# szaguldo-kamaz/FRI-ReinforcementLearning-C

Hardware: AMD Instinct MI355X
Metric: rule-distance evals/sec (rules x envs) (higher is better)
Workload: dtype f64; 1 GPU; cfg4_acrobot_64k_x_8k_per_gpu; nant=5, universe_len=41, rules_per_env=65536, envs_per_gpu=8192, exact_hits=4, dist_backend=none, world_size=1

## Files before the change

fri-reinforcementlearning-c_amd/__init__.py:

```python
import ctypes as C
import os

PKG_DIR = os.path.dirname(os.path.abspath(__file__))
ROOT = os.path.dirname(PKG_DIR)
HIP_LIB_PATH = os.environ.get("FRIRL_HIP_LIB_OVERRIDE") or os.path.join(PKG_DIR, "lib", "libfrirl_hip.so")

NO_HIT = 0xFFFFFFFF
MAX_NANT = 16
MAX_ACTIONS = 32


class FrirlHipError(RuntimeError):
    pass


class Tables(C.Structure):
    _fields_ = [("nant", C.c_int32), ("U", C.c_int32), ("u", C.c_void_p), ("ve", C.c_void_p)]


class RuleBases(C.Structure):
    _fields_ = [("E", C.c_int32), ("maxR", C.c_int32), ("rb", C.c_void_p), ("nrules", C.c_void_p), ("uidx", C.c_void_p)]


MAX_GRID = 64
# ... 77 lines not shown


class AgentIO(C.Structure):
    _fields_ = [("obs", C.c_void_p), ("q_obs", C.c_void_p), ("reward", C.c_void_p), ("success", C.c_void_p), ("reset", C.c_void_p),
                ("action_out", C.c_void_p), ("action_idx", C.c_void_p)]


class DemonstrationDesc(C.Structure):
    _fields_ = [("T", C.c_int32), ("agent_stride", C.c_int64), ("obs", C.c_void_p), ("q_obs", C.c_void_p), ("action", C.c_void_p),
                ("reward", C.c_void_p), ("success", C.c_void_p), ("start", C.c_void_p), ("length", C.c_void_p)]


class PolicyRowsDesc(C.Structure):
    _fields_ = [("Q", C.c_int32), ("done", C.c_void_p), ("ep_steps", C.c_void_p), ("success", C.c_void_p), ("ep_reward", C.c_void_p),
                ("exclude_mask", C.c_void_p), ("rule_slot", C.c_void_p)]


class PolicyBatchRowsDesc(C.Structure):
    _fields_ = [("n", C.c_int32), ("done", C.c_void_p), ("ep_steps", C.c_void_p), ("success", C.c_void_p), ("ep_reward", C.c_void_p),
                ("row_count", C.c_void_p), ("step_cap", C.c_void_p), ("agents", C.c_void_p), ("nagents", C.c_int32),
                ("exclude_mask", C.c_void_p), ("rule_slot", C.c_void_p), ("rows_live", C.c_void_p)]


class ConvergenceDesc(C.Structure):
    _fields_ = [("prev_nrules", C.c_void_p), ("prev_steps", C.c_void_p), ("prev_reward", C.c_void_p), ("prev_rconc", C.c_void_p),
                ("converged", C.c_void_p), ("episodes", C.c_void_p), ("epended", C.c_void_p)]


_lib = None
_DP = C.POINTER(C.c_double)
LEARN_CHUNK_FN = C.CFUNCTYPE(None, C.c_void_p, C.c_int32, C.c_void_p, C.c_int32)

SIGNATURES = {
    "frirl_hip_version": (C.c_char_p, []),
    "frirl_hip_last_error": (C.c_char_p, []),
    "frirl_hip_device_count": (C.c_int, []),
    "frirl_hip_device_info": (C.c_int, [C.c_int, C.c_char_p, C.c_int, C.POINTER(C.c_int32), C.POINTER(C.c_int64)]),
    "frirl_hip_set_option": (C.c_int, [C.c_char_p, C.c_int]),
    "frirl_hip_get_option": (C.c_int, [C.c_char_p, C.POINTER(C.c_int)]),
    "five_hip_rule_distance_uses_uidx": (C.c_int, [C.c_int32, C.c_int32]),
    "frirl_hip_step_uses_uidx": (C.c_int, [C.c_int32, C.c_int32, C.c_int32, C.c_int32]),
    "five_hip_rule_distance": (C.c_int, [C.POINTER(Tables), C.POINTER(RuleBases), C.c_void_p, C.c_void_p, C.c_void_p, C.c_void_p]),
    "five_hip_rule_distance_packed_words": (C.c_int, [C.c_int32, C.c_int32]),
    "frirl_hip_pack_indices": (C.c_int, [C.POINTER(Tables), C.POINTER(RuleBases), C.c_void_p, C.c_void_p]),
    "five_hip_rule_distance_packed": (C.c_int, [C.POINTER(Tables), C.POINTER(RuleBases), C.c_void_p, C.c_void_p, C.c_void_p, C.c_void_p,
                                                C.c_void_p]),
    "five_hip_rule_distance_packed_workspace_bytes": (C.c_size_t, [C.c_int32, C.c_int32, C.c_int32]),
    "five_hip_rule_distance_packed_ws": (C.c_int, [C.POINTER(Tables), C.POINTER(RuleBases), C.c_void_p, C.c_void_p, C.c_void_p, C.c_void_p,
                                                   C.c_void_p, C.c_size_t, C.c_void_p]),
    "five_hip_rule_distance_coded_bytes": (C.c_size_t, [C.c_int32, C.c_int32, C.c_int32, C.c_int32, C.POINTER(C.c_int32)]),
    "frirl_hip_pack_codes": (C.c_int, [C.POINTER(Tables), C.POINTER(RuleBases), C.c_void_p, C.POINTER(C.c_int32), C.c_void_p, C.c_void_p]),
    "five_hip_rule_distance_coded_ws": (C.c_int, [C.POINTER(Tables), C.POINTER(RuleBases), C.c_void_p, C.c_void_p, C.POINTER(C.c_int32), C.c_void_p,
                                                  C.c_void_p, C.c_void_p, C.c_void_p, C.c_void_p, C.c_size_t, C.c_void_p]),
    "five_hip_sqrt_unscaled_check": (C.c_int, [C.c_void_p, C.c_void_p, C.c_void_p, C.c_int64, C.c_void_p]),
    "five_hip_rule_distance_sq_guard": (C.c_int, [C.POINTER(Tables), C.c_int32, C.c_void_p, C.c_void_p, C.c_void_p]),
    "five_hip_vag_concl": (C.c_int, [C.POINTER(Tables), C.POINTER(RuleBases), C.c_int, C.c_void_p, C.c_void_p, C.c_void_p, C.c_void_p]),
    "five_hip_vag_concl_weight": (C.c_int, [C.POINTER(Tables), C.POINTER(RuleBases), C.c_int, C.c_void_p, C.c_void_p, C.c_void_p, C.c_void_p]),
    "frirl_hip_get_best_action": (C.c_int, [C.POINTER(Tables), C.POINTER(RuleBases), C.c_int, C.c_void_p, C.c_void_p, C.c_int,
                                            C.c_void_p, C.c_void_p, C.c_void_p]),
    "five_hip_shepard_weight_check": (C.c_int, [C.c_void_p, C.c_int64, C.c_int, C.c_int, C.c_void_p, C.c_void_p]),
    "frirl_hip_explore_check": (C.c_int, [C.POINTER(AgentDesc), C.c_int64, C.c_void_p, C.c_void_p, C.c_void_p, C.c_void_p, C.c_void_p, C.c_void_p,
                                          C.c_void_p]),
    "five_hip_vag_concl_shared": (C.c_int, [C.POINTER(Tables), C.POINTER(RuleBases), C.c_int, C.c_int32, C.c_void_p, C.c_void_p, C.c_void_p, C.c_void_p]),
    "frirl_hip_get_best_action_shared": (C.c_int, [C.POINTER(Tables), C.POINTER(RuleBases), C.c_int, C.c_int32, C.c_void_p, C.c_void_p, C.c_int,
                                                   C.c_void_p, C.c_void_p, C.c_void_p]),
    "frirl_hip_rollout_shared": (C.c_int, [C.POINTER(Tables), C.POINTER(RuleBases), C.POINTER(AgentDesc), C.c_int32, C.POINTER(RolloutDesc), C.c_void_p]),
    "frirl_hip_rollout_batch_workspace_bytes": (C.c_size_t, [C.c_int32, C.c_int32, C.c_int32, C.c_int32, C.c_int32]),
    "frirl_hip_rollout_batch": (C.c_int, [C.POINTER(Tables), C.POINTER(RuleBases), C.POINTER(AgentDesc), C.POINTER(RolloutBatchDesc), C.c_void_p,
                                          C.c_void_p, C.c_size_t, C.c_void_p]),
    "frirl_hip_rollout_record": (C.c_int, [C.POINTER(Tables), C.POINTER(RuleBases), C.POINTER(AgentDesc), C.POINTER(RolloutLogDesc), C.c_void_p]),
    "frirl_hip_reduce_shared": (C.c_int, [C.POINTER(Tables), C.POINTER(RuleBases), C.POINTER(AgentDesc), C.c_void_p, C.c_int, C.c_double, C.c_int,
                                          C.POINTER(C.c_int32), C.POINTER(ReduceResult), C.c_void_p]),
    "frirl_hip_reduce_batch_depth": (C.c_int, [C.c_int32, C.c_int32]),
    "frirl_hip_reduce_batch_workspace_bytes": (C.c_size_t, [C.c_int32, C.c_int32, C.c_int32, C.c_int32]),
    "frirl_hip_reduce_batch": (C.c_int, [C.POINTER(Tables), C.POINTER(RuleBases), C.POINTER(AgentDesc), C.c_void_p, C.c_void_p, C.c_void_p, C.c_int,
                                         C.c_double, C.c_int, C.POINTER(C.c_int32), C.POINTER(ReduceResult), C.c_void_p, C.c_size_t, C.c_void_p]),
    "frirl_hip_reduce_walk_check": (C.c_int, [C.c_int, C.POINTER(C.c_int32), _DP, C.c_int, C.c_double, C.c_double, C.c_double,
                                              C.POINTER(C.c_uint32), _DP]),
    "frirl_hip_reduce_batch_starts_depth": (C.c_int, [C.c_int32, C.c_int32, C.c_int32]),
    "frirl_hip_reduce_batch_starts_workspace_bytes": (C.c_size_t, [C.c_int32, C.c_int32, C.c_int32, C.c_int32, C.c_int32]),
    "frirl_hip_reduce_batch_starts": (C.c_int, [C.POINTER(Tables), C.POINTER(RuleBases), C.POINTER(AgentDesc), C.c_void_p, C.POINTER(ReduceStarts),
                                                C.c_void_p, C.c_int, C.c_double, C.c_int, C.POINTER(C.c_int32), C.POINTER(ReduceResult),
                                                C.POINTER(ReduceStartResult), C.c_void_p, C.c_size_t, C.c_void_p]),
    "frirl_hip_reduce_walk_starts_check": (C.c_int, [C.c_int, C.c_int, C.POINTER(C.c_int32), _DP, C.POINTER(C.c_int32), _DP, C.c_double, C.c_double,
                                                     C.POINTER(C.c_uint32)]),
    "frirl_hip_lanes_preferred": (C.c_int, [C.c_int32, C.c_int32, C.c_int32]),
    "frirl_hip_lanes_workspace_bytes": (C.c_size_t, [C.c_int32, C.c_int32, C.c_int32, C.c_int32]),
    "frirl_hip_episode_run_lanes": (C.c_int, [C.POINTER(Tables), C.POINTER(RuleBases), C.POINTER(AgentDesc), C.POINTER(EnvsDesc), C.c_int32,
                                              C.c_void_p, C.c_size_t, C.c_void_p]),
    "frirl_hip_rollout_resident_rules": (C.c_int, [C.c_int32, C.c_int32, C.c_int32, C.c_int32]),
    "frirl_hip_learn_supported": (C.c_int, [C.c_int32, C.c_int32, C.c_int32, C.c_int32, C.c_int32]),
    "frirl_hip_learn_plan": (C.c_int, [C.c_int32, C.c_int32, C.POINTER(C.c_int32), C.POINTER(C.c_int32)]),
    "frirl_hip_learn_workspace_bytes": (C.c_size_t, [C.c_int32, C.c_int32, C.c_int32, C.c_int32]),
    "frirl_hip_learn_run": (C.c_int, [C.POINTER(Tables), C.POINTER(RuleBases), C.POINTER(AgentDesc), C.POINTER(EnvsDesc), C.POINTER(ConvergenceDesc),
                                      C.c_void_p, C.c_int32, C.c_int32, C.c_int32, C.c_void_p, C.c_void_p, C.c_void_p, C.c_size_t, C.c_void_p]),
    "frirl_hip_learn_train_workspace_bytes": (C.c_size_t, [C.c_int32, C.c_int32, C.c_int32, C.c_int32]),
    "frirl_hip_learn_train": (C.c_int, [C.POINTER(Tables), C.POINTER(RuleBases), C.POINTER(AgentDesc), C.POINTER(EnvsDesc), C.POINTER(ConvergenceDesc),
                                        C.c_int32, C.c_int32, C.c_void_p, C.c_void_p, C.c_void_p, C.c_void_p, C.c_size_t, C.POINTER(C.c_int32),
                                        LEARN_CHUNK_FN, C.c_void_p, C.c_void_p]),
    "five_hip_add_rule": (C.c_int, [C.POINTER(Tables), C.POINTER(RuleBases), C.c_void_p, C.c_void_p, C.c_void_p, C.c_void_p, C.c_void_p,
                                    C.c_void_p]),
    "frirl_hip_update_sarsa": (C.c_int, [C.POINTER(Tables), C.POINTER(RuleBases), C.POINTER(AgentDesc), C.POINTER(EnvsDesc), C.c_void_p,
                                         C.c_void_p, C.c_void_p, C.c_void_p, C.c_void_p]),
    "frirl_hip_env_step": (C.c_int, [C.POINTER(AgentDesc), C.c_int32, C.c_int32, C.c_void_p, C.c_void_p, C.c_void_p, C.c_void_p, C.c_void_p,
                                     C.c_void_p, C.c_void_p]),
    "frirl_hip_episode_begin": (C.c_int, [C.POINTER(Tables), C.POINTER(RuleBases), C.POINTER(AgentDesc), C.POINTER(EnvsDesc), C.c_void_p]),
# ... 106 lines not shown
            fn = getattr(L, name)
            fn.restype, fn.argtypes = res, args
        _lib = L
    return _lib


def check(rc, what=""):
    if rc != 0:
        raise FrirlHipError(f"{what}: rc={rc}: {lib().frirl_hip_last_error().decode()}")


def set_option(name, value):
    old = C.c_int()
    check(lib().frirl_hip_get_option(name.encode(), C.byref(old)), "frirl_hip_get_option")
    check(lib().frirl_hip_set_option(name.encode(), int(value)), "frirl_hip_set_option")
    return old.value


def _ptr(t):
    return None if t is None else C.c_void_p(t.data_ptr())


def _stream(stream=None):
    import torch
    s = stream if stream is not None else torch.cuda.current_stream()
    return C.c_void_p(s.cuda_stream)


class Problem:

    def __init__(self, u, ve, rb, nrules, uidx=None):
        import torch
        assert u.is_cuda and ve.is_cuda and rb.is_cuda and nrules.is_cuda
        assert u.dtype == torch.float64 and ve.dtype == torch.float64 and rb.dtype == torch.float64 and nrules.dtype == torch.int32
        self.nant, self.U = u.shape
        self.E, cols, self.maxR = rb.shape
        assert cols == self.nant + 1 and ve.shape == u.shape and nrules.shape == (self.E,)
        self.u, self.ve, self.rb, self.nrules = u.contiguous(), ve.contiguous(), rb.contiguous(), nrules.contiguous()
        self.uidx = None
        if uidx is not None:
            assert uidx.is_cuda and uidx.dtype == torch.int16 and uidx.shape == (self.E, self.nant, self.maxR) and self.U <= 32767
            self.uidx = uidx.contiguous()
        self.tables = Tables(self.nant, self.U, self.u.data_ptr(), self.ve.data_ptr())
        self._bases = RuleBases(self.E, self.maxR, self.rb.data_ptr(), self.nrules.data_ptr(),
                                self.uidx.data_ptr() if self.uidx is not None else None)
        self.pidx = None
        self._pidx_key = None
        W = lib().five_hip_rule_distance_packed_words(self.nant, self.U) if self.uidx is not None else 0
        if W > 0:
            self.pidx = torch.empty((self.E, W, self.maxR), dtype=torch.int32, device=self.uidx.device)
            self._pack(None)
        self.codes = self._code_dict = self._code_rank = self._code_d = None
        self._codes_key = None
        if self.pidx is not None and self.nant <= 5:
            self._pack_codes(None)
        self._rd_ws = {}
        self._ro_ws = {}

    @property
    def bases(self):
        self._pidx_key = None
        self._codes_key = None
        return self._bases

    def _pack(self, stream):
        check(lib().frirl_hip_pack_indices(C.byref(self.tables), C.byref(self._bases), _ptr(self.pidx), _stream(stream)),
              "frirl_hip_pack_indices")
        self._pidx_key = (self.uidx.data_ptr(), self.uidx._version)

    def _pidx_current(self, stream):
        if self._pidx_key != (self.uidx.data_ptr(), self.uidx._version):
            self._pack(stream)
        return self.pidx

    def _pack_codes(self, stream):
        import torch
        dev = self.uidx.device
        with torch.cuda.stream(stream if stream is not None else torch.cuda.current_stream()):
            nr = self.nrules.to(torch.int64)
            upto = (nr + (nr & 1)).clamp(max=self.maxR)
            cols = torch.arange(self.maxR, device=dev)
            dimoff = (65 * torch.arange(self.nant, device=dev)).view(1, self.nant, 1)
            counts = torch.zeros((self.nant * 65,), dtype=torch.int64, device=dev)
            step = max(1, (1 << 26) // (self.nant * self.maxR))
            for e0 in range(0, self.E, step):
                v = self.uidx[e0:e0 + step].to(torch.int64) & 63
                live = (cols.view(1, -1) < upto[e0:e0 + step].view(-1, 1)).unsqueeze(1)
                v = torch.where(live, v, torch.full_like(v, 64)) + dimoff
                counts += torch.bincount(v.flatten(), minlength=self.nant * 65)
            present = counts.view(self.nant, 65)[:, :64] > 0
            rank = (present.cumsum(1) - 1).clamp(min=0).to(torch.uint8).contiguous()
            idx = torch.arange(64, device=dev).expand(self.nant, 64)
            dct = torch.where(present, idx, torch.full_like(idx, 255)).sort(1).values.to(torch.uint8).contiguous()
            d = present.sum(1).clamp(min=1).to(torch.int32).cpu().tolist()
        darr = (C.c_int32 * self.nant)(*d)
        n = lib().five_hip_rule_distance_coded_bytes(self.nant, self.U, self.E, self.maxR, darr)
        if n:
            if self.codes is None or self.codes.numel() != n:
                self.codes = torch.empty((n,), dtype=torch.uint8, device=dev)
            self._code_dict, self._code_rank, self._code_d = dct, rank, darr
            check(lib().frirl_hip_pack_codes(C.byref(self.tables), C.byref(self._bases), _ptr(rank), darr, _ptr(self.codes), _stream(stream)),
                  "frirl_hip_pack_codes")
        else:
            self.codes = self._code_dict = self._code_rank = self._code_d = None
        self._codes_key = (self.uidx.data_ptr(), self.uidx._version, self.nrules.data_ptr(), self.nrules._version)

    def _codes_current(self, stream):
        if self.nant <= 5 and self._codes_key != (self.uidx.data_ptr(), self.uidx._version, self.nrules.data_ptr(), self.nrules._version):
            self._pack_codes(stream)
        return self.codes

    def _rd_workspace(self, stream):
        import torch
        key = _stream(stream).value
        if key not in self._rd_ws:
            n = lib().five_hip_rule_distance_packed_workspace_bytes(self.nant, self.U, self.E)
            self._rd_ws[key] = torch.empty((n,), dtype=torch.uint8, device=self.pidx.device) if n else None
        return self._rd_ws[key]

    def rule_distance(self, x, ruledists=None, hit=None, materialise=True, stream=None):
        import torch
        assert x.is_cuda and x.dtype == torch.float64 and x.shape == (self.E, self.nant) and x.is_contiguous()
        if materialise and ruledists is None:
            ruledists = torch.empty((self.E, self.maxR), dtype=torch.float64, device=x.device)
        if hit is None:
            hit = torch.empty((self.E,), dtype=torch.int32, device=x.device)
        if self.pidx is not None and self._codes_current(stream) is not None:
            ws = self._rd_workspace(stream)
            rc = lib().five_hip_rule_distance_coded_ws(C.byref(self.tables), C.byref(self._bases), _ptr(self.codes), _ptr(self._code_dict), self._code_d,
                                                       _ptr(self._pidx_current(stream)), _ptr(x), _ptr(ruledists) if materialise else None,
                                                       _ptr(hit), _ptr(ws), ws.numel() if ws is not None else 0, _stream(stream))
            check(rc, "five_hip_rule_distance_coded_ws")
        elif self.pidx is not None:
            ws = self._rd_workspace(stream)
            rc = lib().five_hip_rule_distance_packed_ws(C.byref(self.tables), C.byref(self._bases), _ptr(self._pidx_current(stream)), _ptr(x),
                                                        _ptr(ruledists) if materialise else None, _ptr(hit), _ptr(ws),
                                                        ws.numel() if ws is not None else 0, _stream(stream))
            check(rc, "five_hip_rule_distance_packed_ws")
        else:
            rc = lib().five_hip_rule_distance(C.byref(self.tables), C.byref(self._bases), _ptr(x),
                                              _ptr(ruledists) if materialise else None, _ptr(hit), _stream(stream))
            check(rc, "five_hip_rule_distance")
        return (ruledists if materialise else None), hit

    def vag_concl(self, x, p=0, stream=None):
        import torch
        assert x.is_cuda and x.dtype == torch.float64 and x.shape == (self.E, self.nant) and x.is_contiguous()
        conc = torch.empty((self.E,), dtype=torch.float64, device=x.device)
        hit = torch.empty((self.E,), dtype=torch.int32, device=x.device)
        check(lib().five_hip_vag_concl(C.byref(self.tables), C.byref(self._bases), p, _ptr(x), _ptr(conc), _ptr(hit), _stream(stream)),
              "five_hip_vag_concl")
        return conc, hit

    def vag_concl_weight(self, x, p=0, weights=None, stream=None):
        import torch
        assert x.is_cuda and x.dtype == torch.float64 and x.shape == (self.E, self.nant) and x.is_contiguous()
        if weights is None:
            weights = torch.full((self.E, self.maxR), float("nan"), dtype=torch.float64, device=x.device)
        hit = torch.empty((self.E,), dtype=torch.int32, device=x.device)
        check(lib().five_hip_vag_concl_weight(C.byref(self.tables), C.byref(self._bases), p, _ptr(x), _ptr(weights), _ptr(hit),
                                              _stream(stream)), "five_hip_vag_concl_weight")
        return weights, hit

    def get_best_action(self, states, action_ve, p=0, stream=None):
        import torch
        assert states.is_cuda and states.dtype == torch.float64 and states.shape == (self.E, self.nant - 1) and states.is_contiguous()
        A = action_ve.numel()
        actconc = torch.empty((self.E, A), dtype=torch.float64, device=states.device)
        best = torch.empty((self.E,), dtype=torch.int32, device=states.device)
        check(lib().frirl_hip_get_best_action(C.byref(self.tables), C.byref(self._bases), p, _ptr(states), _ptr(action_ve), A,
                                              _ptr(actconc), _ptr(best), _stream(stream)), "frirl_hip_get_best_action")
        return actconc, best

    def vag_concl_shared(self, x, p=0, stream=None):
        import torch
        assert self.E == 1 and x.is_cuda and x.dtype == torch.float64 and x.shape[1] == self.nant and x.is_contiguous()
        Q = x.shape[0]
        conc = torch.empty((Q,), dtype=torch.float64, device=x.device)
        hit = torch.empty((Q,), dtype=torch.int32, device=x.device)
        check(lib().five_hip_vag_concl_shared(C.byref(self.tables), C.byref(self._bases), p, Q, _ptr(x), _ptr(conc), _ptr(hit), _stream(stream)),
              "five_hip_vag_concl_shared")
        return conc, hit

    def get_best_action_shared(self, states, action_ve, p=0, stream=None):
        import torch
        assert self.E == 1 and states.is_cuda and states.dtype == torch.float64 and states.shape[1] == self.nant - 1 and states.is_contiguous()
        Q, A = states.shape[0], action_ve.numel()
        actconc = torch.empty((Q, A), dtype=torch.float64, device=states.device)
        best = torch.empty((Q,), dtype=torch.int32, device=states.device)
        check(lib().frirl_hip_get_best_action_shared(C.byref(self.tables), C.byref(self._bases), p, Q, _ptr(states), _ptr(action_ve), A, _ptr(actconc),
                                                     _ptr(best), _stream(stream)), "frirl_hip_get_best_action_shared")
# ... 899 lines not shown
```

fri-reinforcementlearning-c_amd/csrc/five_rule_distance.hip:

```cpp
#include <stdlib.h>

#include <type_traits>

#include "device_common.h"

namespace frirl {

__device__ __forceinline__ void item_to_env_chunk(unsigned item, int cpe, int E, bool env_fastest, int &e, int &c)
{
    if (env_fastest) { c = (int)(item / (unsigned)E); e = (int)(item - (unsigned)c * (unsigned)E); }
    else { e = (int)(item / (unsigned)cpe); c = (int)(item - (unsigned)e * (unsigned)cpe); }
}

template <int NANT, bool WRITE, int UNROLL, int NT>
__global__ __launch_bounds__(FRIRL_BLOCK) void rule_distance_kernel(
    const double *__restrict__ u, const double *__restrict__ ve, int U, const double *__restrict__ rb,
    const int32_t *__restrict__ nrules, int maxR, const double *__restrict__ x, double *__restrict__ dists,
    uint32_t *__restrict__ hit, int rules_per_block, int cpe, int E, int env_fastest)
{
    int e, c;
    item_to_env_chunk(blockIdx.x, cpe, E, env_fastest != 0, e, c);
    const int R = nrules[e];
    const int r0 = c * rules_per_block;
    if (r0 >= R) return;
// ... 959 lines not shown
#pragma unroll
        for (int j = 0; j < 4; j++) {
            const int rr = r + j * STEP;
            if (rr < r_end) {
                const double a0 = cd_rule_sq<NANT>(code[2 * j], sq_s, cs), a1 = cd_rule_sq<NANT>(code[2 * j + 1], sq_s, cs);
                const bool z0 = FAST ? a0 == 0.0 : __dsqrt_rn(a0) == 0.0, z1 = FAST ? a1 == 0.0 : __dsqrt_rn(a1) == 0.0;
                if (z1 && rr + 1 < R) best = min(best, (unsigned)(rr + 1));
                if (z0) best = min(best, (unsigned)rr);
            }
        }
        return best;
    };
    if (any) {
        code[0] = w[0].x << 3;
        code[1] = __builtin_amdgcn_alignbit(w[0].y, w[0].x, 21);
        code[2] = __builtin_amdgcn_alignbit(w[1].x, w[0].y, 13);
        code[3] = w[1].x >> 5;
        code[4] = w[1].y << 3;
        code[5] = __builtin_amdgcn_alignbit(w[2].x, w[1].y, 21);
        code[6] = __builtin_amdgcn_alignbit(w[2].y, w[2].x, 13);
        code[7] = w[2].y >> 5;
        if (fast) sweep(std::true_type{});
        else sweep(std::false_type{});
    }
    if (!__any(lo == 0u)) return;
    unsigned best = FRIRL_HIP_NO_HIT;
    if (any) best = fast ? first_hit(std::true_type{}) : first_hit(std::false_type{});
    best = wave_min_u32(best);
    if ((threadIdx.x & (FRIRL_WAVE - 1)) == 0 && best != FRIRL_HIP_NO_HIT) atomicMin(&hit[e], best);
}

template <int NANT>
static int launch_coded(const frirl_hip_tables *t, const frirl_hip_rulebases *b, const uint8_t *codes, const uint8_t *dict, const CodeParams &cp,
                        const double *x, double *ruledists, uint32_t *hit, void *ws, hipStream_t s)
{
    using namespace frirl_host;
    const long cpe = ((long)b->maxR + RD_CD_TILE - 1) / RD_CD_TILE;
    if (cpe * ((long)b->E + RD_XCDS) > 0x7FFFFFFFL) { set_error("five_hip_rule_distance_coded_ws: too many work items"); return FRIRL_HIP_EINVAL; }
    double *sqtab = static_cast<double *>(ws);
    uint32_t *fastv = reinterpret_cast<uint32_t *>(sqtab + (size_t)b->E * NANT * (1 << RD_PK_BITS));
    const unsigned items = (unsigned)cpe * (unsigned)((b->E + RD_XCDS - 1) / RD_XCDS * RD_XCDS);
    const GroupDiv gd = group_div((uint32_t)(RD_XCDS * cpe));
    hipLaunchKernelGGL((sq_tables_kernel<NANT, RD_PK_BITS, true>), dim3((unsigned)((b->E + FRIRL_WAVES_PER_BLOCK - 1) / FRIRL_WAVES_PER_BLOCK)), dim3(FRIRL_BLOCK),
                       0, s, t->u, t->ve, t->U, b->E, x, sqtab, fastv, hit, dict);
    if (ruledists)
        hipLaunchKernelGGL((rule_distance_cd_kernel<NANT, true>), dim3(items), dim3(FRIRL_BLOCK), 0, s, codes, b->nrules, b->maxR, ruledists, hit, (int)cpe,
                           b->E, sqtab, fastv, cp, gd);
    else
        hipLaunchKernelGGL((rule_distance_cd_kernel<NANT, false>), dim3(items), dim3(FRIRL_BLOCK), 0, s, codes, b->nrules, b->maxR, ruledists, hit, (int)cpe,
                           b->E, sqtab, fastv, cp, gd);
    return check_launch("five_hip_rule_distance_coded_ws");
}

__global__ void sqrt_unscaled_check_kernel(const double *__restrict__ a, double *__restrict__ fast, double *__restrict__ ref, long n)
{
    const long i = (long)blockIdx.x * blockDim.x + threadIdx.x;
    if (i >= n) return;
    fast[i] = sqrt_unscaled(a[i]);
    ref[i] = __dsqrt_rn(a[i]);
}

template <int NANT>
__global__ __launch_bounds__(FRIRL_BLOCK) void sq_guard_kernel(const double *__restrict__ u, const double *__restrict__ ve, int U,
                                                             const double *__restrict__ x, int32_t *__restrict__ ok)
{
    constexpr int TS = 1 << RD_PK_BITS;
    __shared__ double sq_s[NANT * TS];
    __shared__ double q_s[NANT];
    const int e = blockIdx.x;
    double tv[(NANT * TS + FRIRL_BLOCK - 1) / FRIRL_BLOCK];
    load_sq_sources<NANT, RD_PK_BITS, FRIRL_BLOCK>(ve, U, tv, (int)threadIdx.x);
    if (threadIdx.x < NANT) q_s[threadIdx.x] = observe_ve(u, ve, U, threadIdx.x, x[(size_t)e * NANT + threadIdx.x]);
    __syncthreads();
    const bool fast = !__syncthreads_or(!fill_sq_table<NANT, RD_PK_BITS, FRIRL_BLOCK>(q_s, sq_s, tv, (int)threadIdx.x));
    if (threadIdx.x == 0) ok[e] = fast ? 1 : 0;
}

}

extern "C" int five_hip_rule_distance_uses_uidx(int32_t nant, int32_t U)
{
    return nant >= 1 && nant <= FRIRL_HIP_MAX_NANT && U <= 65536 && sizeof(double) * nant * (size_t)U <= 150 * 1024 && !frirl_host::opts().no_uidx;
}

extern "C" int five_hip_rule_distance(const frirl_hip_tables *t, const frirl_hip_rulebases *b, const double *x,
                                      double *ruledists, uint32_t *hit, void *stream)
{
    using namespace frirl_host;
    int rc = check_rulebases(t, b);
    if (rc) return rc;
    if (!x || !hit) { set_error("five_hip_rule_distance: NULL x/hit"); return FRIRL_HIP_EINVAL; }
    if (ruledists && (reinterpret_cast<uintptr_t>(ruledists) & 15)) { set_error("five_hip_rule_distance: ruledists must be 16-byte aligned"); return FRIRL_HIP_EINVAL; }
    if ((rc = check_device())) return rc;
    hipStream_t s = as_stream(stream);

    switch (t->nant) {
#define FRIRL_CASE(N) case N: return frirl::launch_nant<N>(t, b, x, ruledists, hit, s);
        FRIRL_CASE(1) FRIRL_CASE(2) FRIRL_CASE(3) FRIRL_CASE(4) FRIRL_CASE(5) FRIRL_CASE(6) FRIRL_CASE(7) FRIRL_CASE(8)
        FRIRL_CASE(9) FRIRL_CASE(10) FRIRL_CASE(11) FRIRL_CASE(12) FRIRL_CASE(13) FRIRL_CASE(14) FRIRL_CASE(15) FRIRL_CASE(16)
#undef FRIRL_CASE
    }
    set_error("five_hip_rule_distance: unsupported nant=%d", t->nant);
    return FRIRL_HIP_EINVAL;
}

extern "C" int five_hip_rule_distance_packed_words(int32_t nant, int32_t U)
// ... 110 lines not shown
    using namespace frirl_host;
    int rc = check_rulebases(t, b);
    if (rc) return rc;
    if (!b->uidx || !rank || !codes) { set_error("frirl_hip_pack_codes: NULL uidx/rank/codes"); return FRIRL_HIP_EINVAL; }
    frirl::CodeParams cp;
    if (!frirl::coded_bytes(t->nant, t->U, b->E, b->maxR, d) || !frirl::code_params(t->nant, d, cp)) {
        set_error("frirl_hip_pack_codes: nant=%d U=%d with these dictionary lengths is not served by the coded form", t->nant, t->U);
        return FRIRL_HIP_EINVAL;
    }
    if (reinterpret_cast<uintptr_t>(codes) & 7) { set_error("frirl_hip_pack_codes: codes must be 8-byte aligned"); return FRIRL_HIP_EINVAL; }
    if ((rc = check_device())) return rc;
    const int tpe = (b->maxR + frirl::RD_CD_TILE - 1) / frirl::RD_CD_TILE;
    const long ntiles = (long)b->E * tpe;
    long grid = ntiles;
    if (grid > (long)frirl::device_cus() * 32) grid = (long)frirl::device_cus() * 32;
    hipLaunchKernelGGL(frirl::pack_codes_kernel, dim3((unsigned)grid), dim3(FRIRL_BLOCK), 0, as_stream(stream), b->uidx, b->nrules, t->nant, b->maxR, tpe,
                       ntiles, rank, cp, codes);
    return check_launch("frirl_hip_pack_codes");
}

extern "C" int five_hip_rule_distance_coded_ws(const frirl_hip_tables *t, const frirl_hip_rulebases *b, const uint8_t *codes, const uint8_t *dict,
                                               const int32_t *d, const uint32_t *pidx, const double *x, double *ruledists, uint32_t *hit,
                                               void *workspace, size_t workspace_bytes, void *stream)
{
    using namespace frirl_host;
    int rc = check_rulebases(t, b);
    if (rc) return rc;
    const Options &o = opts();
    const bool plain = !o.rd_coded || !o.rd_packed || !o.rd_sqdiff || !o.rd_prepass || o.rd_persist == 1 || o.no_uidx || o.rd_order != 0 ||
                       (o.rd_unroll != 0 && o.rd_unroll != 4) || (o.rd_chunk != 0 && o.rd_chunk != frirl::RD_CD_TILE);
    frirl::CodeParams cp;
    if (plain || !frirl::coded_bytes(t->nant, t->U, b->E, b->maxR, d) || !frirl::code_params(t->nant, d, cp))
        return five_hip_rule_distance_packed_ws(t, b, pidx, x, ruledists, hit, workspace, workspace_bytes, stream);
    const size_t need = frirl::packed_ws_bytes(t->nant, t->U, b->E);
    if (!workspace || workspace_bytes < need) {
        set_error("five_hip_rule_distance_coded_ws: workspace of %zu B at %p, nant=%d U=%d E=%d needs %zu B "
                  "(five_hip_rule_distance_packed_workspace_bytes)", workspace_bytes, workspace, t->nant, t->U, b->E, need);
        return FRIRL_HIP_EINVAL;
    }
    if (reinterpret_cast<uintptr_t>(workspace) & 15) { set_error("five_hip_rule_distance_coded_ws: workspace must be 16-byte aligned"); return FRIRL_HIP_EINVAL; }
    if (!codes || !dict || !x || !hit) { set_error("five_hip_rule_distance_coded_ws: NULL codes/dict/x/hit"); return FRIRL_HIP_EINVAL; }
    if (reinterpret_cast<uintptr_t>(codes) & 7) { set_error("five_hip_rule_distance_coded_ws: codes must be 8-byte aligned"); return FRIRL_HIP_EINVAL; }
    if (ruledists && (reinterpret_cast<uintptr_t>(ruledists) & 15)) { set_error("five_hip_rule_distance_coded_ws: ruledists must be 16-byte aligned"); return FRIRL_HIP_EINVAL; }
    if ((rc = check_device())) return rc;
    hipStream_t s = as_stream(stream);
    switch (t->nant) {
#define FRIRL_CASE(N) case N: return frirl::launch_coded<N>(t, b, codes, dict, cp, x, ruledists, hit, workspace, s);
        FRIRL_CASE(1) FRIRL_CASE(2) FRIRL_CASE(3) FRIRL_CASE(4) FRIRL_CASE(5)
#undef FRIRL_CASE
    }
    set_error("five_hip_rule_distance_coded_ws: unsupported nant=%d", t->nant);
    return FRIRL_HIP_EINVAL;
}
```

include/frirl_hip.h:

```cpp
#ifndef FRIRL_HIP_H
#define FRIRL_HIP_H

#include <stdint.h>

#ifdef __cplusplus
extern "C" {
#endif

#define FRIRL_HIP_MAX_NANT     16
#define FRIRL_HIP_MAX_ACTIONS  32
#define FRIRL_HIP_MAX_GRID     64
#define FRIRL_HIP_NO_HIT       0xFFFFFFFFu

#define FRIRL_HIP_ENV_MOUNTAINCAR 0
#define FRIRL_HIP_ENV_CARTPOLE    1
#define FRIRL_HIP_ENV_ACROBOT     2
#define FRIRL_HIP_ENV_EXTERNAL    3

#define FRIRL_HIP_UPD_INACTIVE   0
#define FRIRL_HIP_UPD_EXACT      1
#define FRIRL_HIP_UPD_SPREAD     2
#define FRIRL_HIP_UPD_INSERTED   3
#define FRIRL_HIP_UPD_SKIPPED    4
#define FRIRL_HIP_UPD_FULL       5

#define FRIRL_HIP_OK        0
#define FRIRL_HIP_ENODEV   -1
#define FRIRL_HIP_EINVAL   -2
#define FRIRL_HIP_ELAUNCH  -3

typedef struct frirl_hip_tables {
    int32_t nant;
    int32_t U;
    const double *u;
    const double *ve;
} frirl_hip_tables;

typedef struct frirl_hip_rulebases {
    int32_t E;
    int32_t maxR;
    double *rb;
    int32_t *nrules;
    uint16_t *uidx;
} frirl_hip_rulebases;

const char *frirl_hip_version(void);
const char *frirl_hip_last_error(void);
int frirl_hip_device_count(void);
int frirl_hip_device_info(int device, char *name, int name_len, int32_t *cus, int64_t *hbm_bytes);

int frirl_hip_set_option(const char *name, int value);
int frirl_hip_get_option(const char *name, int *value);
int five_hip_rule_distance_uses_uidx(int32_t nant, int32_t U);
int frirl_hip_step_uses_uidx(int32_t nant, int32_t U, int32_t maxR, int32_t E);

int five_hip_rule_distance(const frirl_hip_tables *t, const frirl_hip_rulebases *b, const double *x,
                           double *ruledists, uint32_t *hit, void *stream);

int five_hip_rule_distance_packed_words(int32_t nant, int32_t U);
int frirl_hip_pack_indices(const frirl_hip_tables *t, const frirl_hip_rulebases *b, uint32_t *pidx, void *stream);
int five_hip_rule_distance_packed(const frirl_hip_tables *t, const frirl_hip_rulebases *b, const uint32_t *pidx, const double *x,
                                  double *ruledists, uint32_t *hit, void *stream);
size_t five_hip_rule_distance_packed_workspace_bytes(int32_t nant, int32_t U, int32_t E);
int five_hip_rule_distance_packed_ws(const frirl_hip_tables *t, const frirl_hip_rulebases *b, const uint32_t *pidx, const double *x,
                                     double *ruledists, uint32_t *hit, void *workspace, size_t workspace_bytes, void *stream);
size_t five_hip_rule_distance_coded_bytes(int32_t nant, int32_t U, int32_t E, int32_t maxR, const int32_t *d);
int frirl_hip_pack_codes(const frirl_hip_tables *t, const frirl_hip_rulebases *b, const uint8_t *rank, const int32_t *d, uint8_t *codes,
                         void *stream);
int five_hip_rule_distance_coded_ws(const frirl_hip_tables *t, const frirl_hip_rulebases *b, const uint8_t *codes, const uint8_t *dict,
                                    const int32_t *d, const uint32_t *pidx, const double *x, double *ruledists, uint32_t *hit,
                                    void *workspace, size_t workspace_bytes, void *stream);
int five_hip_sqrt_unscaled_check(const double *a, double *fast, double *ref, int64_t n, void *stream);
int five_hip_rule_distance_sq_guard(const frirl_hip_tables *t, int32_t E, const double *x, int32_t *ok, void *stream);

int five_hip_vag_concl(const frirl_hip_tables *t, const frirl_hip_rulebases *b, int p, const double *x,
                       double *conc, uint32_t *hit, void *stream);

int five_hip_vag_concl_weight(const frirl_hip_tables *t, const frirl_hip_rulebases *b, int p, const double *x,
                              double *weights, uint32_t *hit, void *stream);

int frirl_hip_get_best_action(const frirl_hip_tables *t, const frirl_hip_rulebases *b, int p, const double *states,
                              const double *action_ve, int A, double *actconc, int32_t *best, void *stream);

int five_hip_shepard_weight_check(const double *s, int64_t n, int p, int form, double *w, void *stream);

typedef struct frirl_hip_agent {
    double alpha, gamma;
    double qdiff_pos_boundary;
    double qdiff_neg_boundary;
    double weight_significant;
    int32_t skip_rules;
    int32_t p;
    int32_t A;
    int32_t env_kind;
    int32_t max_steps;
    int32_t no_random;
    int32_t grid_len[FRIRL_HIP_MAX_NANT];
    double grid_div[FRIRL_HIP_MAX_NANT];
    double values_def[FRIRL_HIP_MAX_NANT];
    const double *grid_values;
    const double *action_ve;
    double epsilon;
    double reward_good_above;
    double qdiff_final_tolerance;
    uint64_t seed;
    int32_t evaluate;
    int32_t debug_flags;
    uint64_t env_id_base;
} frirl_hip_agent;

int frirl_hip_explore_check(const frirl_hip_agent *agent, int64_t n, const uint32_t *env, const uint32_t *episode, const uint32_t *step,
                            const int32_t *greedy, int32_t *out_action, double *out_unit, void *stream);

typedef struct frirl_hip_rollout {
    const double *start_states;
    const uint32_t *exclude_mask;
    const uint8_t *rule_slot;
    int32_t *steps;
    double *reward;
    int32_t *success;
    double *final_states;
} frirl_hip_rollout;
int frirl_hip_rollout_shared(const frirl_hip_tables *t, const frirl_hip_rulebases *b, const frirl_hip_agent *agent, int32_t Q,
                             const frirl_hip_rollout *ro, void *stream);
// ... 349 lines not shown
```

Measured before the change: 545.5 billion evals/s.

## Add wide dictionary-coded rule-distance path for larger per-dimension tables

Adds a new coded form for rule bases whose value tables exceed the small-table limit. Each rule's per-dimension dictionary ranks are packed into 48-bit codes, three 64-bit words per thread covering four rules. A persistent kernel with an atomic work counter and a prefetched next item reads these codes and looks up distances from an LDS table. The aim is to shrink the bytes streamed per rule compared with int16 index reads. The cost is an extra packing kernel, a per-call hipMallocAsync, and more dispatch complexity; it only applies when the table size falls in the wide window and the earlier packed path is not taken.

```diff
diff --git a/fri-reinforcementlearning-c_amd/__init__.py b/fri-reinforcementlearning-c_amd/__init__.py
--- a/fri-reinforcementlearning-c_amd/__init__.py
+++ b/fri-reinforcementlearning-c_amd/__init__.py
@@ -153,6 +153,11 @@
     "frirl_hip_pack_codes": (C.c_int, [C.POINTER(Tables), C.POINTER(RuleBases), C.c_void_p, C.POINTER(C.c_int32), C.c_void_p, C.c_void_p]),
     "five_hip_rule_distance_coded_ws": (C.c_int, [C.POINTER(Tables), C.POINTER(RuleBases), C.c_void_p, C.c_void_p, C.POINTER(C.c_int32), C.c_void_p,
                                                   C.c_void_p, C.c_void_p, C.c_void_p, C.c_void_p, C.c_size_t, C.c_void_p]),
+    "five_hip_rule_distance_wide_bytes": (C.c_size_t, [C.c_int32, C.c_int32, C.c_int32, C.c_int32, C.POINTER(C.c_int32)]),
+    "five_hip_rule_distance_wide_fields": (C.c_int, [C.c_int32, C.c_int32, C.POINTER(C.c_int32), C.POINTER(C.c_uint32), C.POINTER(C.c_uint32)]),
+    "frirl_hip_pack_wide": (C.c_int, [C.POINTER(Tables), C.POINTER(RuleBases), C.c_void_p, C.POINTER(C.c_int32), C.c_void_p, C.c_void_p]),
+    "five_hip_rule_distance_wide": (C.c_int, [C.POINTER(Tables), C.POINTER(RuleBases), C.c_void_p, C.c_void_p, C.POINTER(C.c_int32), C.c_void_p,
+                                              C.c_void_p, C.c_void_p, C.c_void_p]),
     "five_hip_sqrt_unscaled_check": (C.c_int, [C.c_void_p, C.c_void_p, C.c_void_p, C.c_int64, C.c_void_p]),
     "five_hip_rule_distance_sq_guard": (C.c_int, [C.POINTER(Tables), C.c_int32, C.c_void_p, C.c_void_p, C.c_void_p]),
     "five_hip_vag_concl": (C.c_int, [C.POINTER(Tables), C.POINTER(RuleBases), C.c_int, C.c_void_p, C.c_void_p, C.c_void_p, C.c_void_p]),
@@ -365,6 +370,8 @@
             self._pack(None)
         self.codes = self._code_dict = self._code_rank = self._code_d = None
         self._codes_key = None
+        ones = (C.c_int32 * self.nant)(*([1] * self.nant))
+        self._wide = self.uidx is not None and lib().five_hip_rule_distance_wide_bytes(self.nant, self.U, self.E, self.maxR, ones) > 0
         if self.pidx is not None and self.nant <= 5:
             self._pack_codes(None)
         self._rd_ws = {}
@@ -389,31 +396,35 @@
     def _pack_codes(self, stream):
         import torch
         dev = self.uidx.device
+        W = self.U if self._wide else 64
+        small, none = (torch.int16, 0x7FFF) if self._wide else (torch.uint8, 255)
         with torch.cuda.stream(stream if stream is not None else torch.cuda.current_stream()):
             nr = self.nrules.to(torch.int64)
             upto = (nr + (nr & 1)).clamp(max=self.maxR)
             cols = torch.arange(self.maxR, device=dev)
-            dimoff = (65 * torch.arange(self.nant, device=dev)).view(1, self.nant, 1)
-            counts = torch.zeros((self.nant * 65,), dtype=torch.int64, device=dev)
+            dimoff = ((W + 1) * torch.arange(self.nant, device=dev)).view(1, self.nant, 1)
+            counts = torch.zeros((self.nant * (W + 1),), dtype=torch.int64, device=dev)
             step = max(1, (1 << 26) // (self.nant * self.maxR))
             for e0 in range(0, self.E, step):
-                v = self.uidx[e0:e0 + step].to(torch.int64) & 63
+                v = self.uidx[e0:e0 + step].to(torch.int64)
+                v = v.clamp(0, W - 1) if self._wide else v & 63
                 live = (cols.view(1, -1) < upto[e0:e0 + step].view(-1, 1)).unsqueeze(1)
-                v = torch.where(live, v, torch.full_like(v, 64)) + dimoff
-                counts += torch.bincount(v.flatten(), minlength=self.nant * 65)
-            present = counts.view(self.nant, 65)[:, :64] > 0
-            rank = (present.cumsum(1) - 1).clamp(min=0).to(torch.uint8).contiguous()
-            idx = torch.arange(64, device=dev).expand(self.nant, 64)
-            dct = torch.where(present, idx, torch.full_like(idx, 255)).sort(1).values.to(torch.uint8).contiguous()
+                v = torch.where(live, v, torch.full_like(v, W)) + dimoff
+                counts += torch.bincount(v.flatten(), minlength=self.nant * (W + 1))
+            present = counts.view(self.nant, W + 1)[:, :W] > 0
+            rank = (present.cumsum(1) - 1).clamp(min=0).to(small).contiguous()
+            idx = torch.arange(W, device=dev).expand(self.nant, W)
+            dct = torch.where(present, idx, torch.full_like(idx, none)).sort(1).values.to(small).contiguous()
             d = present.sum(1).clamp(min=1).to(torch.int32).cpu().tolist()
         darr = (C.c_int32 * self.nant)(*d)
-        n = lib().five_hip_rule_distance_coded_bytes(self.nant, self.U, self.E, self.maxR, darr)
+        size, pack = ((lib().five_hip_rule_distance_wide_bytes, lib().frirl_hip_pack_wide) if self._wide else
+                      (lib().five_hip_rule_distance_coded_bytes, lib().frirl_hip_pack_codes))
+        n = size(self.nant, self.U, self.E, self.maxR, darr)
         if n:
             if self.codes is None or self.codes.numel() != n:
                 self.codes = torch.empty((n,), dtype=torch.uint8, device=dev)
             self._code_dict, self._code_rank, self._code_d = dct, rank, darr
-            check(lib().frirl_hip_pack_codes(C.byref(self.tables), C.byref(self._bases), _ptr(rank), darr, _ptr(self.codes), _stream(stream)),
-                  "frirl_hip_pack_codes")
+            check(pack(C.byref(self.tables), C.byref(self._bases), _ptr(rank), darr, _ptr(self.codes), _stream(stream)), pack.__name__)
         else:
             self.codes = self._code_dict = self._code_rank = self._code_d = None
         self._codes_key = (self.uidx.data_ptr(), self.uidx._version, self.nrules.data_ptr(), self.nrules._version)
@@ -450,6 +461,10 @@
                                                         _ptr(ruledists) if materialise else None, _ptr(hit), _ptr(ws),
                                                         ws.numel() if ws is not None else 0, _stream(stream))
             check(rc, "five_hip_rule_distance_packed_ws")
+        elif self._wide and self._codes_current(stream) is not None:
+            rc = lib().five_hip_rule_distance_wide(C.byref(self.tables), C.byref(self._bases), _ptr(self.codes), _ptr(self._code_dict), self._code_d,
+                                                   _ptr(x), _ptr(ruledists) if materialise else None, _ptr(hit), _stream(stream))
+            check(rc, "five_hip_rule_distance_wide")
         else:
             rc = lib().five_hip_rule_distance(C.byref(self.tables), C.byref(self._bases), _ptr(x),
                                               _ptr(ruledists) if materialise else None, _ptr(hit), _stream(stream))
diff --git a/fri-reinforcementlearning-c_amd/csrc/five_rule_distance.hip b/fri-reinforcementlearning-c_amd/csrc/five_rule_distance.hip
--- a/fri-reinforcementlearning-c_amd/csrc/five_rule_distance.hip
+++ b/fri-reinforcementlearning-c_amd/csrc/five_rule_distance.hip
@@ -1035,6 +1035,224 @@
     return check_launch("five_hip_rule_distance_coded_ws");
 }
 
+static constexpr int RD_WD_BLOCK = 512, RD_WD_TILE = 2 * RD_WD_BLOCK * 2, RD_WD_TILE_BYTES = 6 * RD_WD_TILE, RD_WD_PIECE = 8 * RD_WD_BLOCK;
+static constexpr int RD_WD_MAX_NANT = 5, RD_WD_MAX_BITS = 48;
+
+struct WideParams {
+    uint32_t shift[RD_WD_MAX_NANT], bits[RD_WD_MAX_NANT], d[RD_WD_MAX_NANT];
+};
+
+static bool wide_shape(int nant, int U)
+{
+    if (nant < 1 || nant > RD_WD_MAX_NANT || U < 1) return false;
+    const size_t tab_bytes = sizeof(double) * (size_t)nant * (size_t)U;
+    return tab_bytes > RD_SMALL_TABLE_BYTES && tab_bytes <= 64 * 1024;
+}
+
+static int wide_params(int nant, int U, const int32_t *d, WideParams &wp)
+{
+    if (!wide_shape(nant, U) || !d) return 0;
+    int total = 0, na = 0;
+    for (int k = 0; k < RD_WD_MAX_NANT; k++) wp.shift[k] = wp.bits[k] = 0u, wp.d[k] = 1u;
+    for (int k = 0; k < nant; k++) {
+        if (d[k] < 1 || d[k] > U) return 0;
+        const int bits = ceil_log2((uint32_t)d[k]);
+        wp.shift[k] = (uint32_t)total;
+        wp.bits[k] = (uint32_t)bits;
+        wp.d[k] = (uint32_t)d[k];
+        total += bits;
+        if (total <= 32) na = k + 1;
+    }
+    return total <= RD_WD_MAX_BITS ? na : 0;
+}
+
+static size_t wide_bytes(int nant, int U, long E, long maxR, const int32_t *d)
+{
+    WideParams wp;
+    if (E < 1 || maxR < 2 || !wide_params(nant, U, d, wp)) return 0;
+    return (size_t)E * (size_t)((maxR + RD_WD_TILE - 1) / RD_WD_TILE) * RD_WD_TILE_BYTES;
+}
+
+__global__ __launch_bounds__(RD_WD_BLOCK) void pack_wide_kernel(const uint16_t *__restrict__ uidx, const int32_t *__restrict__ nrules, int nant, int U, int maxR,
+                                                                int tpe, long ntiles, const uint16_t *__restrict__ rank, WideParams wp,
+                                                                uint8_t *__restrict__ codes)
+{
+    const int t = threadIdx.x;
+    for (long tile = blockIdx.x; tile < ntiles; tile += gridDim.x) {
+        const long e = tile / tpe;
+        const int c = (int)(tile - e * tpe);
+        const int R = nrules[e];
+        const int Rp = min(R + (R & 1), maxR);
+        const uint16_t *__restrict__ src = uidx + (size_t)e * nant * maxR;
+        uint64_t code[4];
+#pragma unroll
+        for (int i = 0; i < 4; i++) {
+            const int r = c * RD_WD_TILE + 2 * t + (i & 1) + 2 * RD_WD_BLOCK * (i >> 1);
+            uint64_t v = 0u;
+            if (r < Rp) {
+                for (int k = 0; k < nant; k++) {
+                    const uint32_t i_k = min((uint32_t)src[(size_t)k * maxR + r], (uint32_t)(U - 1));
+                    v |= (uint64_t)rank[k * U + i_k] << wp.shift[k];
+                }
+            }
+            code[i] = v & ((1ull << RD_WD_MAX_BITS) - 1ull);
+        }
+        uint64_t *__restrict__ dst = reinterpret_cast<uint64_t *>(codes + (size_t)tile * RD_WD_TILE_BYTES + 8 * t);
+        dst[0] = code[0] | code[1] << 48;
+        dst[RD_WD_PIECE / 8] = code[1] >> 16 | code[2] << 32;
+        dst[2 * (RD_WD_PIECE / 8)] = code[2] >> 32 | code[3] << 16;
+    }
+}
+
+template <int NANT, int NA>
+struct WideScan {
+    uint32_t off[NANT], bits[NANT];
+    __device__ __forceinline__ explicit WideScan(const WideParams &wp)
+    {
+#pragma unroll
+        for (int k = 0; k < NANT; k++) off[k] = k < NA ? wp.shift[k] : wp.shift[k] - 16u, bits[k] = wp.bits[k];
+    }
+};
+
+template <int NANT, int NA>
+__device__ __forceinline__ double2 wide_pair_distance(uint32_t a0, uint32_t b0, uint32_t a1, uint32_t b1, const double (&q)[NANT],
+                                                      const double *__restrict__ tab_s, int U, const WideScan<NANT, NA> &ws)
+{
+    double a0s = 0.0, a1s = 0.0;
+#pragma unroll
+    for (int k = 0; k < NANT; k++) {
+        const double *__restrict__ row = tab_s + k * U;
+        const double t0 = row[__builtin_amdgcn_ubfe(k < NA ? a0 : b0, ws.off[k], ws.bits[k])];
+        const double t1 = row[__builtin_amdgcn_ubfe(k < NA ? a1 : b1, ws.off[k], ws.bits[k])];
+        const double d0 = q[k] - t0, d1 = q[k] - t1;
+        const double s0 = d0 * d0, s1 = d1 * d1;
+        a0s = k == 0 ? s0 : a0s + s0;
+        a1s = k == 0 ? s1 : a1s + s1;
+    }
+    double2 d;
+    d.x = __dsqrt_rn(a0s);
+    d.y = __dsqrt_rn(a1s);
+    return d;
+}
+
+template <int NANT, int NA, bool WRITE>
+__global__ __launch_bounds__(RD_WD_BLOCK) void rule_distance_wide_persist_kernel(
+    const double *__restrict__ ve, int U, const uint16_t *__restrict__ dict, const uint8_t *__restrict__ codes, const int32_t *__restrict__ nrules,
+    int maxR, const double *__restrict__ qv, double *__restrict__ dists, uint32_t *__restrict__ hit, int cpe, int nitems,
+    unsigned *__restrict__ counter, WideParams wp)
+{
+    extern __shared__ double tab_s[];
+    __shared__ int batch_s[2];
+    constexpr int BLOCK = RD_WD_BLOCK, KB = 4, STEP = BLOCK * 2;
+    const int nbatches = (nitems + KB - 1) / KB;
+    u32x2_t w[3];
+    double qn[NANT];
+    int en = 0, cn = 0, Rn = 0;
+    auto load_item = [&](int it) {
+        en = it / cpe; cn = it - en * cpe;
+        Rn = nrules[en];
+        if (cn * RD_WD_TILE + 2 * (int)threadIdx.x < Rn) {
+            const uint8_t *__restrict__ src = codes + (size_t)it * RD_WD_TILE_BYTES + 8 * threadIdx.x;
+#pragma unroll
+            for (int m = 0; m < 3; m++) w[m] = __builtin_nontemporal_load(reinterpret_cast<const u32x2_t *>(src + m * RD_WD_PIECE));
+        }
+#pragma unroll
+        for (int k = 0; k < NANT; k++) qn[k] = qv[(size_t)en * NANT + k];
+    };
+    int slot = 0, sub = 0;
+    if (threadIdx.x == 0) batch_s[0] = (int)atomicAdd(counter, 1u);
+    __syncthreads();
+    int batch = batch_s[0];
+    int item = batch < nbatches ? batch * KB : nitems;
+    if (item < nitems) load_item(item);
+#pragma unroll
+    for (int k = 0; k < NANT; k++)
+        for (int j = threadIdx.x; j < (int)wp.d[k]; j += BLOCK) tab_s[k * U + j] = ve[k * U + min((int)dict[k * U + j], U - 1)];
+    const WideScan<NANT, NA> ws(wp);
+    __syncthreads();
+    while (item < nitems) {
+        const int e = en, c = cn, R = Rn;
+        u32x2_t cw[3];
+        double q[NANT];
+#pragma unroll
+        for (int m = 0; m < 3; m++) cw[m] = w[m];
+#pragma unroll
+        for (int k = 0; k < NANT; k++) q[k] = qn[k];
+        int nxt;
+        sub++;
+        if (sub < KB && item + 1 < nitems) nxt = item + 1;
+        else {
+            sub = 0;
+            slot ^= 1;
+            if (threadIdx.x == 0) batch_s[slot] = (int)atomicAdd(counter, 1u);
+            __syncthreads();
+            batch = batch_s[slot];
+            nxt = batch < nbatches ? batch * KB : nitems;
+        }
+        if (nxt < nitems) load_item(nxt);
+        double *__restrict__ out = WRITE ? dists + (size_t)e * maxR : nullptr;
+        const int r = c * RD_WD_TILE + 2 * (int)threadIdx.x;
+        unsigned best = FRIRL_HIP_NO_HIT;
+#pragma unroll
+        for (int j = 0; j < 2; j++) {
+            const int rr = r + j * STEP;
+            if (rr < R) {
+                const uint32_t x0 = j == 0 ? cw[0].x : cw[1].y, x1 = j == 0 ? cw[0].y : cw[2].x, x2 = j == 0 ? cw[1].x : cw[2].y;
+                const double2 d = wide_pair_distance<NANT, NA>(x0, __builtin_amdgcn_alignbit(x1, x0, 16), __builtin_amdgcn_alignbit(x2, x1, 16), x2,
+                                                               q, tab_s, U, ws);
+                if (WRITE) { __builtin_nontemporal_store(d.x, out + rr); __builtin_nontemporal_store(d.y, out + rr + 1); }
+                if (d.y == 0.0 && rr + 1 < R) best = min(best, (unsigned)(rr + 1));
+                if (d.x == 0.0) best = min(best, (unsigned)rr);
+            }
+        }
+        if (best != FRIRL_HIP_NO_HIT) atomicMin(&hit[e], best);
+        item = nxt;
+    }
+}
+
+template <int NANT, int NA>
+static int launch_wide(const frirl_hip_tables *t, const frirl_hip_rulebases *b, const uint8_t *codes, const uint16_t *dict, const WideParams &wp,
+                       const double *x, double *ruledists, uint32_t *hit, hipStream_t s)
+{
+    using namespace frirl_host;
+    const size_t tab_bytes = sizeof(double) * NANT * (size_t)t->U;
+    const long cpe = ((long)b->maxR + RD_WD_TILE - 1) / RD_WD_TILE;
+    const long nitems = cpe * (long)b->E;
+    if (nitems > 0x7FFFFFF0L) { set_error("five_hip_rule_distance_wide: %ld work items exceed the 31-bit item index", nitems); return FRIRL_HIP_EINVAL; }
+    const long nbatches = (nitems + 3) / 4;
+    const int wgs = 3 * (tab_bytes + 256) <= 160 * 1024 ? 3 : 2;
+    long grid = (long)device_cus() * wgs;
+    if (grid > nbatches) grid = nbatches;
+    const size_t qv_off = 256, bytes = qv_off + sizeof(double) * (size_t)b->E * NANT;
+    void *scratch = nullptr;
+    hipError_t e1 = hipMallocAsync(&scratch, bytes, s);
+    if (e1 != hipSuccess) { (void)hipGetLastError(); set_error("five_hip_rule_distance_wide: hipMallocAsync(%zu B) failed: %s", bytes, hipGetErrorString(e1)); return FRIRL_HIP_ELAUNCH; }
+    unsigned *counter = static_cast<unsigned *>(scratch);
+    double *qv = reinterpret_cast<double *>(static_cast<char *>(scratch) + qv_off);
+    const int nq = b->E * NANT;
+    hipLaunchKernelGGL(observe_reset_kernel, dim3((nq + 255) / 256), dim3(256), 0, s, t->u, t->ve, t->U, NANT, b->E, x, qv, hit, counter);
+    auto launch = [&](auto k) {
+        e1 = hipFuncSetAttribute(reinterpret_cast<const void *>(k), hipFuncAttributeMaxDynamicSharedMemorySize, (int)tab_bytes);
+        if (e1 == hipSuccess) hipLaunchKernelGGL(k, dim3((unsigned)grid), dim3(RD_WD_BLOCK), tab_bytes, s, t->ve, t->U, dict, codes, b->nrules, b->maxR, qv, ruledists, hit, (int)cpe, (int)nitems, counter, wp);
+    };
+    if (ruledists) launch(rule_distance_wide_persist_kernel<NANT, NA, true>);
+    else launch(rule_distance_wide_persist_kernel<NANT, NA, false>);
+    const hipError_t e2 = hipFreeAsync(scratch, s);
+    if (e1 != hipSuccess) { set_error("five_hip_rule_distance_wide: cannot reserve %zu B of LDS: %s", tab_bytes, hipGetErrorString(e1)); return FRIRL_HIP_ELAUNCH; }
+    if (e2 != hipSuccess) { set_error("five_hip_rule_distance_wide: hipFreeAsync failed: %s", hipGetErrorString(e2)); return FRIRL_HIP_ELAUNCH; }
+    return check_launch("five_hip_rule_distance_wide");
+}
+
+template <int NANT, int NA = NANT>
+static int launch_wide_na(int na, const frirl_hip_tables *t, const frirl_hip_rulebases *b, const uint8_t *codes, const uint16_t *dict, const WideParams &wp,
+                          const double *x, double *ruledists, uint32_t *hit, hipStream_t s)
+{
+    if (na == NA) return launch_wide<NANT, NA>(t, b, codes, dict, wp, x, ruledists, hit, s);
+    if constexpr (NA > 1) return launch_wide_na<NANT, NA - 1>(na, t, b, codes, dict, wp, x, ruledists, hit, s);
+    frirl_host::set_error("five_hip_rule_distance_wide: no field in the low word");
+    return FRIRL_HIP_EINVAL;
+}
+
 __global__ void sqrt_unscaled_check_kernel(const double *__restrict__ a, double *__restrict__ fast, double *__restrict__ ref, long n)
 {
     const long i = (long)blockIdx.x * blockDim.x + threadIdx.x;
@@ -1251,3 +1469,67 @@
     set_error("five_hip_rule_distance_coded_ws: unsupported nant=%d", t->nant);
     return FRIRL_HIP_EINVAL;
 }
+
+extern "C" size_t five_hip_rule_distance_wide_bytes(int32_t nant, int32_t U, int32_t E, int32_t maxR, const int32_t *d)
+{
+    return frirl::wide_bytes(nant, U, E, maxR, d);
+}
+
+extern "C" int five_hip_rule_distance_wide_fields(int32_t nant, int32_t U, const int32_t *d, uint32_t *shift, uint32_t *mask)
+{
+    frirl::WideParams wp;
+    if (!frirl::wide_params(nant, U, d, wp)) return -1;
+    for (int k = 0; k < nant; k++) {
+        if (shift) shift[k] = wp.shift[k];
+        if (mask) mask[k] = (1u << wp.bits[k]) - 1u;
+    }
+    return (int)(wp.shift[nant - 1] + wp.bits[nant - 1]);
+}
+
+extern "C" int frirl_hip_pack_wide(const frirl_hip_tables *t, const frirl_hip_rulebases *b, const uint16_t *rank, const int32_t *d, uint8_t *codes,
+                                   void *stream)
+{
+    using namespace frirl_host;
+    int rc = check_rulebases(t, b);
+    if (rc) return rc;
+    if (!b->uidx || !rank || !codes) { set_error("frirl_hip_pack_wide: NULL uidx/rank/codes"); return FRIRL_HIP_EINVAL; }
+    frirl::WideParams wp;
+    if (!frirl::wide_bytes(t->nant, t->U, b->E, b->maxR, d) || !frirl::wide_params(t->nant, t->U, d, wp)) {
+        set_error("frirl_hip_pack_wide: nant=%d U=%d with these dictionary lengths is not served by the wide coded form", t->nant, t->U);
+        return FRIRL_HIP_EINVAL;
+    }
+    if (reinterpret_cast<uintptr_t>(codes) & 7) { set_error("frirl_hip_pack_wide: codes must be 8-byte aligned"); return FRIRL_HIP_EINVAL; }
+    if ((rc = check_device())) return rc;
+    const int tpe = (b->maxR + frirl::RD_WD_TILE - 1) / frirl::RD_WD_TILE;
+    const long ntiles = (long)b->E * tpe;
+    long grid = ntiles;
+    if (grid > (long)frirl::device_cus() * 16) grid = (long)frirl::device_cus() * 16;
+    hipLaunchKernelGGL(frirl::pack_wide_kernel, dim3((unsigned)grid), dim3(frirl::RD_WD_BLOCK), 0, as_stream(stream), b->uidx, b->nrules, t->nant, t->U,
+                       b->maxR, tpe, ntiles, rank, wp, codes);
+    return check_launch("frirl_hip_pack_wide");
+}
+
+extern "C" int five_hip_rule_distance_wide(const frirl_hip_tables *t, const frirl_hip_rulebases *b, const uint8_t *codes, const uint16_t *dict,
+                                           const int32_t *d, const double *x, double *ruledists, uint32_t *hit, void *stream)
+{
+    using namespace frirl_host;
+    int rc = check_rulebases(t, b);
+    if (rc) return rc;
+    const Options &o = opts();
+    frirl::WideParams wp;
+    const int na = (!o.rd_coded || o.no_uidx || o.rd_persist == 0 || !frirl::wide_bytes(t->nant, t->U, b->E, b->maxR, d)) ? 0
+                                                                                                                            : frirl::wide_params(t->nant, t->U, d, wp);
+    if (!na) return five_hip_rule_distance(t, b, x, ruledists, hit, stream);
+    if (!codes || !dict || !x || !hit) { set_error("five_hip_rule_distance_wide: NULL codes/dict/x/hit"); return FRIRL_HIP_EINVAL; }
+    if (reinterpret_cast<uintptr_t>(codes) & 7) { set_error("five_hip_rule_distance_wide: codes must be 8-byte aligned"); return FRIRL_HIP_EINVAL; }
+    if (ruledists && (reinterpret_cast<uintptr_t>(ruledists) & 15)) { set_error("five_hip_rule_distance_wide: ruledists must be 16-byte aligned"); return FRIRL_HIP_EINVAL; }
+    if ((rc = check_device())) return rc;
+    hipStream_t s = as_stream(stream);
+    switch (t->nant) {
+#define FRIRL_CASE(N) case N: return frirl::launch_wide_na<N>(na, t, b, codes, dict, wp, x, ruledists, hit, s);
+        FRIRL_CASE(1) FRIRL_CASE(2) FRIRL_CASE(3) FRIRL_CASE(4) FRIRL_CASE(5)
+#undef FRIRL_CASE
+    }
+    set_error("five_hip_rule_distance_wide: unsupported nant=%d", t->nant);
+    return FRIRL_HIP_EINVAL;
+}
diff --git a/include/frirl_hip.h b/include/frirl_hip.h
--- a/include/frirl_hip.h
+++ b/include/frirl_hip.h
@@ -70,6 +70,12 @@
 int five_hip_rule_distance_coded_ws(const frirl_hip_tables *t, const frirl_hip_rulebases *b, const uint8_t *codes, const uint8_t *dict,
                                     const int32_t *d, const uint32_t *pidx, const double *x, double *ruledists, uint32_t *hit,
                                     void *workspace, size_t workspace_bytes, void *stream);
+size_t five_hip_rule_distance_wide_bytes(int32_t nant, int32_t U, int32_t E, int32_t maxR, const int32_t *d);
+int five_hip_rule_distance_wide_fields(int32_t nant, int32_t U, const int32_t *d, uint32_t *shift, uint32_t *mask);
+int frirl_hip_pack_wide(const frirl_hip_tables *t, const frirl_hip_rulebases *b, const uint16_t *rank, const int32_t *d, uint8_t *codes,
+                        void *stream);
+int five_hip_rule_distance_wide(const frirl_hip_tables *t, const frirl_hip_rulebases *b, const uint8_t *codes, const uint16_t *dict,
+                                const int32_t *d, const double *x, double *ruledists, uint32_t *hit, void *stream);
 int five_hip_sqrt_unscaled_check(const double *a, double *fast, double *ref, int64_t n, void *stream);
 int five_hip_rule_distance_sq_guard(const frirl_hip_tables *t, int32_t E, const double *x, int32_t *ok, void *stream);
 
```

After: 523.4 billion evals/s. 0.959x the previous value.
